# Ajax0564/VyomAI

Measured on AMD Instinct MI355X. Metric: training tokens/sec (12L d=768 seq=512 GPT-style decoder, CLM), higher is better.
Workload: dtype bf16; 1 GPU; configs[1]: GPT-style Decoder 12L d=768 h=12 RoPE vocab 50265, CLM training B=32/GPU seq=512, AdamW, bf16 kernels + fp32 masters; global_batch=32, seq_len=512, parallelism=dp1, attention=none, weights=deterministic recipe (vyomai_amd.recipe)

## Files before the change

### vyomai_amd/csrc/vy_misc.hip

```cpp
#include "vy_common.h"
#include <stdarg.h>
#include <string.h>

static thread_local char g_err[512] = "";
void vy_set_error(const char* fmt, ...) {
  va_list ap;
  va_start(ap, fmt);
  vsnprintf(g_err, sizeof(g_err), fmt, ap);
  va_end(ap);
}
extern "C" const char* vy_last_error(void) { return g_err; }
extern "C" int vy_abi_version(void) { return 5; }

namespace {

template <typename T, int CH>
__global__ __launch_bounds__(256) void layernorm_fwd_kernel(const T* __restrict__ x, int64_t ldx,
                                                            const T* __restrict__ gamma,
                                                            const T* __restrict__ beta, T* __restrict__ y,
                                                            int64_t ldy, float* __restrict__ mean_out,
                                                            float* __restrict__ rstd_out, int64_t M, int N,
                                                            float eps) {
  constexpr int VEC = Chunk<T>::VEC;
  const int lane = threadIdx.x & 63;
  const int64_t row = (int64_t)blockIdx.x * 4 + (threadIdx.x >> 6);
  if (row >= M) return;
  const int nch = N / VEC;
  float v[CH][VEC];
  float s = 0.f;
#pragma unroll
  for (int c = 0; c < CH; ++c) {
    const int ch = lane + 64 * c;
    if (ch < nch) {
      Chunk<T>::load(x + row * ldx + (int64_t)ch * VEC, v[c]);
#pragma unroll
      for (int e = 0; e < VEC; ++e) s += v[c][e];
    } else {
#pragma unroll
      for (int e = 0; e < VEC; ++e) v[c][e] = 0.f;
    }
  }
  const float mean = vy_wave_sum(s) / (float)N;
  float q = 0.f;
#pragma unroll
  for (int c = 0; c < CH; ++c) {
    const int ch = lane + 64 * c;
    if (ch < nch) {
#pragma unroll
      for (int e = 0; e < VEC; ++e) { const float d = v[c][e] - mean; q += d * d; }
    }
  }
  const float var = vy_wave_sum(q) / (float)N;
  const float rstd = rsqrtf(var + eps);
  const float rstd_r = rstd * (1.5f - 0.5f * (var + eps) * rstd * rstd);
#pragma unroll
  for (int c = 0; c < CH; ++c) {
    const int ch = lane + 64 * c;
    if (ch < nch) {
      float g[VEC], b[VEC], o[VEC];
      Chunk<T>::load(gamma + (int64_t)ch * VEC, g);
      Chunk<T>::load(beta + (int64_t)ch * VEC, b);
#pragma unroll
      for (int e = 0; e < VEC; ++e) o[e] = (v[c][e] - mean) * rstd_r * g[e] + b[e];
      Chunk<T>::store(y + row * ldy + (int64_t)ch * VEC, o);
    }
  }
  if (lane == 0) {
    if (mean_out) mean_out[row] = mean;
    if (rstd_out) rstd_out[row] = rstd_r;
  }
}

template <typename T, int CH>
__global__ __launch_bounds__(256) void rmsnorm_fwd_kernel(const T* __restrict__ x, int64_t ldx,
                                                          const T* __restrict__ w, T* __restrict__ y, int64_t ldy,
                                                          int64_t M, int N, float eps, float w_offset) {
  constexpr int VEC = Chunk<T>::VEC;
  const int lane = threadIdx.x & 63;
  const int64_t row = (int64_t)blockIdx.x * 4 + (threadIdx.x >> 6);
  if (row >= M) return;
  const int nch = N / VEC;
  float v[CH][VEC];
  float q = 0.f;
#pragma unroll
  for (int c = 0; c < CH; ++c) {
    const int ch = lane + 64 * c;
    if (ch < nch) {
      Chunk<T>::load(x + row * ldx + (int64_t)ch * VEC, v[c]);
#pragma unroll
      for (int e = 0; e < VEC; ++e) q += v[c][e] * v[c][e];
    }
  }
  const float ms = vy_wave_sum(q) / (float)N + eps;
  float r = rsqrtf(ms);
  r = r * (1.5f - 0.5f * ms * r * r);
#pragma unroll
  for (int c = 0; c < CH; ++c) {
    const int ch = lane + 64 * c;
    if (ch < nch) {
      float g[VEC], o[VEC];
      Chunk<T>::load(w + (int64_t)ch * VEC, g);
#pragma unroll
      for (int e = 0; e < VEC; ++e) o[e] = v[c][e] * r * (w_offset + g[e]);
      Chunk<T>::store(y + row * ldy + (int64_t)ch * VEC, o);
    }
  }
}

template <typename T, int ACT>
__global__ void gated_act_kernel(const T* __restrict__ gu, int64_t ldg, T* __restrict__ out, int64_t ldo,
                                 int64_t M, int I, int code) {
  constexpr int VEC = Chunk<T>::VEC;
  const int nch = I / VEC;
  const int64_t total = M * nch;
  vy_act_dispatch<ACT>(code, [&](auto a_) {
    constexpr int A = decltype(a_)::value;
    for (int64_t i = (int64_t)blockIdx.x * blockDim.x + threadIdx.x; i < total; i += (int64_t)gridDim.x * blockDim.x) {
      const int64_t m = i / nch;
      const int c = (int)(i - m * nch) * VEC;
      float a[VEC], b[VEC], o[VEC];
      Chunk<T>::load(gu + m * ldg + c, a);
      Chunk<T>::load(gu + m * ldg + I + c, b);
#pragma unroll
      for (int e = 0; e < VEC; ++e) {
        if constexpr (ACT == VY_ACT_RUNTIME && sizeof(T) == 2) o[e] = vy_act_fwd_fast<A>(a[e]) * b[e];
        else o[e] = vy_act_fwd<A>(a[e]) * b[e];
      }
      Chunk<T>::store(out + m * ldo + c, o);
    }
  });
}

template <typename T, int CH>
__global__ __launch_bounds__(256) void layernorm_bwd_kernel(
    const T* __restrict__ dy, int64_t lddy, const T* __restrict__ x, int64_t ldx,
    const T* __restrict__ gamma, const float* __restrict__ mean, const float* __restrict__ rstd,
    T* __restrict__ dx, int64_t lddx, float* __restrict__ ws, int64_t M, int N, int W) {
  constexpr int VEC = Chunk<T>::VEC;
  const int lane = threadIdx.x & 63;
  const int wid = blockIdx.x * 4 + (threadIdx.x >> 6);
  const int nch = N / VEC;
  float g[CH][VEC], dg[CH][VEC], db[CH][VEC];
#pragma unroll
  for (int c = 0; c < CH; ++c) {
    const int ch = lane + 64 * c;
#pragma unroll
    for (int e = 0; e < VEC; ++e) { dg[c][e] = 0.f; db[c][e] = 0.f; g[c][e] = 0.f; }
    if (ch < nch) Chunk<T>::load(gamma + (int64_t)ch * VEC, g[c]);
  }
  typedef typename Chunk<T>::Raw Raw;
  Raw xr[CH], dr[CH], xn[CH], dn[CH];
  float mu = 0.f, rs = 0.f, mu_n = 0.f, rs_n = 0.f;
  auto fetch = [&](int64_t row, Raw (&xa)[CH], Raw (&da)[CH], float& m_, float& r_) {
    m_ = mean[row]; r_ = rstd[row];
#pragma unroll
    for (int c = 0; c < CH; ++c) {
      const int ch = lane + 64 * c;
      if (ch < nch) {
        xa[c] = *reinterpret_cast<const Raw*>(x + row * ldx + (int64_t)ch * VEC);
        da[c] = *reinterpret_cast<const Raw*>(dy + row * lddy + (int64_t)ch * VEC);
      }
    }
  };
  if (wid < M) fetch(wid, xr, dr, mu, rs);
  for (int64_t row = wid; row < M; row += W) {
    const bool more = row + W < M;
    if (more) fetch(row + W, xn, dn, mu_n, rs_n);
    float xh[CH][VEC], gy[CH][VEC];
    float s1 = 0.f, s2 = 0.f;
#pragma unroll
    for (int c = 0; c < CH; ++c) {
      const int ch = lane + 64 * c;
      if (ch < nch) {
        float xv[VEC], dv[VEC];
        Chunk<T>::unpack(xr[c], xv);
        Chunk<T>::unpack(dr[c], dv);
#pragma unroll
        for (int e = 0; e < VEC; ++e) {
          xh[c][e] = (xv[e] - mu) * rs;
          gy[c][e] = dv[e] * g[c][e];
          s1 += gy[c][e];
          s2 += gy[c][e] * xh[c][e];
          dg[c][e] += dv[e] * xh[c][e];
          db[c][e] += dv[e];
        }
      }
    }
    s1 = vy_wave_sum(s1) / (float)N;
    s2 = vy_wave_sum(s2) / (float)N;
#pragma unroll
    for (int c = 0; c < CH; ++c) {
      const int ch = lane + 64 * c;
      if (ch < nch) {
        float o[VEC];
#pragma unroll
        for (int e = 0; e < VEC; ++e) o[e] = rs * (gy[c][e] - s1 - xh[c][e] * s2);
        Chunk<T>::store(dx + row * lddx + (int64_t)ch * VEC, o);
      }
    }
    if (more) {
#pragma unroll
      for (int c = 0; c < CH; ++c) { xr[c] = xn[c]; dr[c] = dn[c]; }
      mu = mu_n; rs = rs_n;
    }
  }
  __shared__ float red[2][3][64 * CH * VEC];
  const int wv = threadIdx.x >> 6;
  if (wv > 0) {
#pragma unroll
    for (int c = 0; c < CH; ++c)
#pragma unroll
      for (int e = 0; e < VEC; ++e) {
        red[0][wv - 1][(c * VEC + e) * 64 + lane] = dg[c][e];
        red[1][wv - 1][(c * VEC + e) * 64 + lane] = db[c][e];
      }
  }
  __syncthreads();
  if (wv != 0) return;
  const int WB = W / 4;
  float* wg = ws + (int64_t)blockIdx.x * N;
  float* wb = ws + (int64_t)WB * N + (int64_t)blockIdx.x * N;
#pragma unroll
  for (int c = 0; c < CH; ++c) {
    const int ch = lane + 64 * c;
    if (ch < nch) {
#pragma unroll
      for (int e = 0; e < VEC; ++e) {
        float a = dg[c][e], b = db[c][e];
#pragma unroll
        for (int w2 = 0; w2 < 3; ++w2) {
          a += red[0][w2][(c * VEC + e) * 64 + lane];
          b += red[1][w2][(c * VEC + e) * 64 + lane];
        }
        wg[ch * VEC + e] = a; wb[ch * VEC + e] = b;
      }
    }
  }
}

__global__ __launch_bounds__(256) void colsum_partials_kernel(float* __restrict__ ws, int W, int N,
                                                              float* __restrict__ out0, float* __restrict__ out1,
                                                              int rows_per_slice, int acc) {
  __shared__ float red[2][4][64];
  const int c = threadIdx.x & 63, g = threadIdx.x >> 6;
  const int n = blockIdx.x * 64 + c;
  const int w0 = blockIdx.y * rows_per_slice, w1 = min(W, w0 + rows_per_slice);
  float a = 0.f, b = 0.f;
  if (n < N) {
    for (int wb = w0 + g; wb < w1; wb += 32) {
      float av[8], bv[8];
#pragma unroll
      for (int i = 0; i < 8; ++i) {
        const int w = wb + 4 * i;
        const int wc = w < w1 ? w : wb;
        av[i] = ws[(int64_t)wc * N + n];
        bv[i] = ws[(int64_t)(W + wc) * N + n];
      }
#pragma unroll
      for (int i = 0; i < 8; ++i)
        if (wb + 4 * i < w1) { a += av[i]; b += bv[i]; }
    }
  }
  red[0][g][c] = a; red[1][g][c] = b;
  __syncthreads();
  if (g == 0 && n < N && w0 < w1) {
    a = red[0][0][c] + red[0][1][c] + red[0][2][c] + red[0][3][c];
    b = red[1][0][c] + red[1][1][c] + red[1][2][c] + red[1][3][c];
    if (gridDim.y == 1) {
      if (out0) out0[n] = (acc ? out0[n] : 0.f) + a;
      if (out1) out1[n] = (acc ? out1[n] : 0.f) + b;
    } else {
      ws[(int64_t)w0 * N + n] = a;
      ws[(int64_t)(W + w0) * N + n] = b;
    }
  }
}

__global__ __launch_bounds__(256) void colsum_finish_kernel(const float* __restrict__ ws, int W, int N,
                                                            float* __restrict__ out0, float* __restrict__ out1,
                                                            int rows_per_slice, int acc) {
  const int n = blockIdx.x * 256 + threadIdx.x;
  if (n >= N) return;
  float a = 0.f, b = 0.f;
  for (int w = 0; w < W; w += rows_per_slice) {
    a += ws[(int64_t)w * N + n];
    b += ws[(int64_t)(W + w) * N + n];
  }
  if (out0) out0[n] = (acc ? out0[n] : 0.f) + a;
  if (out1) out1[n] = (acc ? out1[n] : 0.f) + b;
}

template <typename T>
__device__ __forceinline__ float rl(float x) { return x; }
template <>
__device__ __forceinline__ float rl<bf16>(float x) { return vy_round_bf16(x); }

template <typename T>
__global__ void rope_kernel(T* __restrict__ x, int64_t sb, int64_t sh, int64_t sl,
                            const float* __restrict__ cos_tab, const float* __restrict__ sin_tab,
                            int64_t pos0, int64_t B, int heads, int64_t L, int dh, int inverse) {
  const int half = dh >> 1;
  const int64_t idx = (int64_t)blockIdx.x * blockDim.x + threadIdx.x;
  const int64_t total = B * heads * L * half;
  if (idx >= total) return;
  const int i = (int)(idx % half);
  int64_t r = idx / half;
  const int64_t l = r % L; r /= L;
  const int hd = (int)(r % heads);
  const int64_t b = r / heads;
  T* p = x + b * sb + hd * sh + l * sl;
  const float c = rl<T>(cos_tab[(pos0 + l) * half + i]);
  float s = rl<T>(sin_tab[(pos0 + l) * half + i]);
  if (inverse) s = -s;
  const float a = VyT<T>::ld(p + i), bb = VyT<T>::ld(p + i + half);
  VyT<T>::st(p + i, rl<T>(a * c) + rl<T>(-bb * s));
  VyT<T>::st(p + i + half, rl<T>(bb * c) + rl<T>(a * s));
}

template <typename T>
__global__ void rope2_kernel(T* __restrict__ xq, int64_t q_sb, int64_t q_sh, int64_t q_sl, int hq,
                             T* __restrict__ xk, int64_t k_sb, int64_t k_sh, int64_t k_sl, int hk,
                             const float* __restrict__ cos_tab, const float* __restrict__ sin_tab,
                             int64_t pos0, int64_t B, int64_t L, int dh) {
  const bool isk = blockIdx.y == 1;
  T* x = isk ? xk : xq;
  const int64_t sb = isk ? k_sb : q_sb, sh = isk ? k_sh : q_sh, sl = isk ? k_sl : q_sl;
  const int heads = isk ? hk : hq;
  const int half = dh >> 1;
  const int64_t idx = (int64_t)blockIdx.x * blockDim.x + threadIdx.x;
  if (idx >= B * heads * L * half) return;
  const int i = (int)(idx % half);
  int64_t r = idx / half;
  const int64_t l = r % L; r /= L;
  const int hd = (int)(r % heads);
  const int64_t b = r / heads;
  T* p = x + b * sb + hd * sh + l * sl;
  const float c = rl<T>(cos_tab[(pos0 + l) * half + i]);
  const float s = rl<T>(sin_tab[(pos0 + l) * half + i]);
  const float a = VyT<T>::ld(p + i), bb = VyT<T>::ld(p + i + half);
  VyT<T>::st(p + i, rl<T>(a * c) + rl<T>(-bb * s));
  VyT<T>::st(p + i + half, rl<T>(bb * c) + rl<T>(a * s));
}

template <typename S, typename D>
__global__ void cast_kernel(const S* __restrict__ src, D* __restrict__ dst, int64_t n) {
  int64_t i = ((int64_t)blockIdx.x * blockDim.x + threadIdx.x) * 4;
  const int64_t stride = (int64_t)gridDim.x * blockDim.x * 4;
  for (; i < n; i += stride) {
#pragma unroll
    for (int e = 0; e < 4; ++e)
      if (i + e < n) dst[i + e] = (D)(float)src[i + e];
  }
}

template <typename T>
__global__ void transpose_kernel(const T* __restrict__ in, int64_t ldin, T* __restrict__ out, int64_t ldout,
// ... 284 lines not shown
    float v[VEC], o[VEC];
    Chunk<T>::load(row + (int64_t)c * VEC, v);
#pragma unroll
    for (int e = 0; e < VEC; ++e) {
      const int col = c * VEC + e;
      float g = 0.f;
      if (!dead && col < V) g = p.grad(s, __expf(v[e] - l), col == label ? 1.f : 0.f);
      o[e] = g;
    }
    Chunk<T>::store(row + (int64_t)c * VEC, o);
  }
}

template <typename P>
__global__ __launch_bounds__(1024) void row_fused_kernel(bf16* __restrict__ logits, int64_t ld,
                                                         const int64_t* __restrict__ labels, const P p,
                                                         float* __restrict__ lse, int V, int* __restrict__ err) {
  constexpr int CPT = 8;
  __shared__ float red[16];
  const int tid = threadIdx.x;
  const int64_t m = blockIdx.x;
  const int64_t label = labels[m];
  const auto s = p.load(m, true);
  bf16* row = logits + m * ld;
  const int nch = (V + 7) / 8;
  bf16x8 zero8;
#pragma unroll
  for (int e = 0; e < 8; ++e) zero8[e] = (bf16)0.f;
  const bool live = p.live(s, label);
  const bool oob = live && (label < 0 || label >= V);
  if (oob && err && tid == 0) *err = 1;
  if (!live || oob) {
    for (int c = tid; c < nch; c += 1024) *reinterpret_cast<bf16x8*>(row + (int64_t)c * 8) = zero8;
    if (tid == 0) { lse[m] = 0.f; p.skip(m); }
    return;
  }
  const float x_label = (float)row[label];
  bf16x8 v[CPT];
#pragma unroll
  for (int i = 0; i < CPT; ++i) {
    const int c = tid + i * 1024;
    if (c < nch) v[i] = *reinterpret_cast<const bf16x8*>(row + (int64_t)c * 8);
  }
  float mx = -INFINITY;
#pragma unroll
  for (int i = 0; i < CPT; ++i) {
    const int c = tid + i * 1024;
    if (c < nch) {
#pragma unroll
      for (int e = 0; e < 8; ++e)
        if (c * 8 + e < V) mx = fmaxf(mx, (float)v[i][e]);
    }
  }
  if constexpr (P::kSample) {
    __shared__ RowBest redb[16];
    RowBest best{-INFINITY, INT32_MAX};
#pragma unroll
    for (int i = 0; i < CPT; ++i) {
      const int c = tid + i * 1024;
      if (c < nch) {
        float f[8];
        Chunk<bf16>::unpack(v[i], f);
        p.template scan<8>(m, c, f, V, best);
      }
    }
    const RowBest g = block_argmax(best, redb);
    if (tid == 0) p.sampled(m, g.col);
  }
  const float gmx = block_reduce(mx, red, true);
  float sm = 0.f;
#pragma unroll
  for (int i = 0; i < CPT; ++i) {
    const int c = tid + i * 1024;
    if (c < nch) {
#pragma unroll
      for (int e = 0; e < 8; ++e)
        if (c * 8 + e < V) sm += __expf((float)v[i][e] - gmx);
    }
  }
  const float gsm = block_reduce(sm, red, false);
  const float l = gmx + __logf(gsm);
  if (tid == 0) {
    lse[m] = l;
    p.emit(m, l, x_label);
  }
#pragma unroll
  for (int i = 0; i < CPT; ++i) {
    const int c = tid + i * 1024;
    if (c < nch) {
      bf16x8 o;
#pragma unroll
      for (int e = 0; e < 8; ++e) {
        const int col = c * 8 + e;
        float g = 0.f;
        if (col < V) g = p.grad(s, __expf((float)v[i][e] - l), col == label ? 1.f : 0.f);
        o[e] = (bf16)g;
      }
      *reinterpret_cast<bf16x8*>(row + (int64_t)c * 8) = o;
    }
  }
}

int row_check(const char* fn, bool ptrs, const void* logits, int64_t ld, int64_t M, int64_t V, int dtype, const char* pair) {
  if (!ptrs || M <= 0 || V <= 0) VY_FAIL(VY_ERR_ARG, "%s: bad arguments", fn);
  if (pair) {
    if (dtype != VY_BF16) VY_FAIL(VY_ERR_UNSUPPORTED, "%s: bf16 only (use %s)", fn, pair);
    if (V > 65536) VY_FAIL(VY_ERR_UNSUPPORTED, "%s: V=%ld exceeds the 65536 columns a workgroup keeps in registers (use %s)", fn, (long)V, pair);
    if (ld % 8 || ld < vy_cdiv(V, 8) * 8 || (uintptr_t)logits % 16) VY_FAIL(VY_ERR_ARG, "%s: rows must be 16-byte aligned and cover the padded width", fn);
    return VY_OK;
  }
  const int vec = dtype == VY_BF16 ? 8 : 4;
  if (ld % vec || ld < vy_cdiv(V, vec) * vec) VY_FAIL(VY_ERR_ARG, "%s: row stride must be a multiple of %d and cover the padded row", fn, vec);
  if (dtype != VY_BF16 && dtype != VY_F32) VY_FAIL(VY_ERR_ARG, "%s: bad dtype %d", fn, dtype);
  return VY_OK;
}

template <typename P>
int row_lse(const char* fn, bool ptrs, const void* logits, int64_t ld, const int64_t* labels, const P& p, float* lse,
            int64_t M, int64_t V, int32_t* err, int dtype, void* stream) {
  if (const int rc = row_check(fn, ptrs && logits && labels && lse, logits, ld, M, V, dtype, nullptr)) return rc;
  const dim3 grid((unsigned)M), block(256);
  if (dtype == VY_BF16) hipLaunchKernelGGL((row_lse_kernel<bf16, P>), grid, block, 0, (hipStream_t)stream, (const bf16*)logits, ld, labels, p, lse, (int)V, err);
  else hipLaunchKernelGGL((row_lse_kernel<float, P>), grid, block, 0, (hipStream_t)stream, (const float*)logits, ld, labels, p, lse, (int)V, err);
  VY_CHECK_LAUNCH(fn);
  return VY_OK;
}

template <typename P>
int row_grad(const char* fn, bool ptrs, void* logits, int64_t ld, const int64_t* labels, const P& p, const float* lse,
             int64_t M, int64_t V, int dtype, void* stream) {
  if (const int rc = row_check(fn, ptrs && logits && labels && lse, logits, ld, M, V, dtype, nullptr)) return rc;
  const dim3 grid((unsigned)M), block(256);
  if (dtype == VY_BF16) hipLaunchKernelGGL((row_grad_kernel<bf16, P>), grid, block, 0, (hipStream_t)stream, (bf16*)logits, ld, labels, p, lse, (int)V);
  else hipLaunchKernelGGL((row_grad_kernel<float, P>), grid, block, 0, (hipStream_t)stream, (float*)logits, ld, labels, p, lse, (int)V);
  VY_CHECK_LAUNCH(fn);
  return VY_OK;
}

template <typename P>
int row_fused(const char* fn, bool ptrs, void* logits, int64_t ld, const int64_t* labels, const P& p, float* lse,
              int64_t M, int64_t V, int32_t* err, int dtype, void* stream) {
  if (const int rc = row_check(fn, ptrs && logits && labels && lse, logits, ld, M, V, dtype, P::kPair)) return rc;
  hipLaunchKernelGGL((row_fused_kernel<P>), dim3((unsigned)M), dim3(1024), 0, (hipStream_t)stream, (bf16*)logits, ld, labels, p, lse, (int)V, err);
  VY_CHECK_LAUNCH(fn);
  return VY_OK;
}

template <typename T>
int ln_fwd_dispatch(const void* x, int64_t ldx, const void* gamma, const void* beta, void* y, int64_t ldy,
                    float* mean, float* rstd, int64_t M, int64_t N, float eps, hipStream_t st) {
  constexpr int VEC = Chunk<T>::VEC;
  if (N % VEC || ldx % VEC || ldy % VEC) VY_FAIL(VY_ERR_ARG, "vy_layernorm_fwd: N/ld must be multiples of %d", VEC);
  const int nch = (int)(N / VEC);
  const dim3 grid((unsigned)vy_cdiv(M, 4)), block(256);
#define LN_GO(CH)                                                                                       \
  hipLaunchKernelGGL((layernorm_fwd_kernel<T, CH>), grid, block, 0, st, (const T*)x, ldx, (const T*)gamma, \
                     (const T*)beta, (T*)y, ldy, mean, rstd, M, (int)N, eps)
  if (nch <= 64) LN_GO(1);
  else if (nch <= 128) LN_GO(2);
  else if (nch <= 256) LN_GO(4);
  else if (nch <= 512) LN_GO(8);
  else if (nch <= 1024) LN_GO(16);
  else VY_FAIL(VY_ERR_UNSUPPORTED, "vy_layernorm_fwd: N=%ld too wide", (long)N);
#undef LN_GO
  VY_CHECK_LAUNCH("vy_layernorm_fwd");
  return VY_OK;
}

template <typename T>
int ln_bwd_dispatch(const void* dy, int64_t lddy, const void* x, int64_t ldx, const void* gamma,
                    const float* mean, const float* rstd, void* dx, int64_t lddx, float* dgamma,
                    float* dbeta, float beta, float* ws, int64_t M, int64_t N, hipStream_t st, bool partial = false) {
  constexpr int VEC = Chunk<T>::VEC;
  if (N % VEC || ldx % VEC || lddy % VEC || lddx % VEC) VY_FAIL(VY_ERR_ARG, "vy_layernorm_bwd: N/ld must be multiples of %d", VEC);
  const int nch = (int)(N / VEC);
  const int WB = (int)vy_layernorm_bwd_ws_rows(M);
  const int W = WB * 4;
  const dim3 grid((unsigned)WB), block(256);
#define LN_GO(CH)                                                                                        \
  hipLaunchKernelGGL((layernorm_bwd_kernel<T, CH>), grid, block, 0, st, (const T*)dy, lddy, (const T*)x, ldx, \
                     (const T*)gamma, mean, rstd, (T*)dx, lddx, ws, M, (int)N, W)
  if (nch <= 64) LN_GO(1);
  else if (nch <= 128) LN_GO(2);
  else if (nch <= 256) LN_GO(4);
  else VY_FAIL(VY_ERR_UNSUPPORTED, "vy_layernorm_bwd: N=%ld too wide", (long)N);
#undef LN_GO
  VY_CHECK_LAUNCH("vy_layernorm_bwd");
  if (partial) return VY_OK;
  if (beta != 0.f && beta != 1.f) VY_FAIL(VY_ERR_ARG, "vy_layernorm_bwd: beta must be 0 or 1");
  return vy_ln_colsum(ws, WB, (int)N, dgamma, dbeta, beta == 1.f, st);
}

}

int vy_ln_colsum(float* ws, int WB, int N, float* dgamma, float* dbeta, int acc, hipStream_t st) {
  const int slices = vy_ln_colsum_slices(WB);
  const int rps = (int)vy_cdiv(WB, slices);
  hipLaunchKernelGGL(colsum_partials_kernel, dim3((unsigned)vy_cdiv(N, 64), (unsigned)slices), dim3(256), 0, st, ws, WB,
                     N, dgamma, dbeta, rps, acc);
  VY_CHECK_LAUNCH("vy_layernorm_bwd(colsum)");
  if (slices > 1) {
    hipLaunchKernelGGL(colsum_finish_kernel, dim3((unsigned)vy_cdiv(N, 256)), dim3(256), 0, st, ws, WB, N, dgamma,
                       dbeta, rps, acc);
    VY_CHECK_LAUNCH("vy_layernorm_bwd(colsum finish)");
  }
  return VY_OK;
}

extern "C" int vy_layernorm_fwd(const void* x, int64_t ldx, const void* gamma, const void* beta, void* y,
                                int64_t ldy, float* mean, float* rstd, int64_t M, int64_t N, float eps,
                                int dtype, void* stream) {
  if (!x || !gamma || !beta || !y || M <= 0 || N <= 0) VY_FAIL(VY_ERR_ARG, "vy_layernorm_fwd: bad arguments");
  hipStream_t st = (hipStream_t)stream;
  if (dtype == VY_BF16) return ln_fwd_dispatch<bf16>(x, ldx, gamma, beta, y, ldy, mean, rstd, M, N, eps, st);
  if (dtype == VY_F32) return ln_fwd_dispatch<float>(x, ldx, gamma, beta, y, ldy, mean, rstd, M, N, eps, st);
  VY_FAIL(VY_ERR_ARG, "vy_layernorm_fwd: bad dtype %d", dtype);
}

extern "C" int vy_rmsnorm_fwd(const void* x, int64_t ldx, const void* w, void* y, int64_t ldy, int64_t M, int64_t N,
                              float eps, float w_offset, int dtype, void* stream) {
  if (!x || !w || !y || M <= 0 || N <= 0) VY_FAIL(VY_ERR_ARG, "vy_rmsnorm_fwd: bad arguments");
  hipStream_t st = (hipStream_t)stream;
  const int vec = dtype == VY_BF16 ? 8 : 4;
  if (N % vec || ldx % vec || ldy % vec) VY_FAIL(VY_ERR_ARG, "vy_rmsnorm_fwd: N/ld must be multiples of %d", vec);
  const int nch = (int)(N / vec);
  const dim3 grid((unsigned)vy_cdiv(M, 4)), block(256);
#define RMS_GO(T, CH) hipLaunchKernelGGL((rmsnorm_fwd_kernel<T, CH>), grid, block, 0, st, (const T*)x, ldx, (const T*)w, (T*)y, ldy, M, (int)N, eps, w_offset)
#define RMS_DISPATCH(T)                                  \
  if (nch <= 64) RMS_GO(T, 1);                           \
  else if (nch <= 128) RMS_GO(T, 2);                     \
  else if (nch <= 256) RMS_GO(T, 4);                     \
  else if (nch <= 512) RMS_GO(T, 8);                     \
  else if (nch <= 1024) RMS_GO(T, 16);                   \
  else VY_FAIL(VY_ERR_UNSUPPORTED, "vy_rmsnorm_fwd: N=%ld too wide", (long)N)
  if (dtype == VY_BF16) { RMS_DISPATCH(bf16); }
  else if (dtype == VY_F32) { RMS_DISPATCH(float); }
  else VY_FAIL(VY_ERR_ARG, "vy_rmsnorm_fwd: bad dtype %d", dtype);
#undef RMS_DISPATCH
#undef RMS_GO
  VY_CHECK_LAUNCH("vy_rmsnorm_fwd");
  return VY_OK;
}

extern "C" int vy_gated_act_fwd(const void* gate_up, int64_t ldg, void* out, int64_t ldo, int64_t M, int64_t I, int act,
                                int dtype, void* stream) {
  if (!gate_up || !out || M <= 0 || I <= 0) VY_FAIL(VY_ERR_ARG, "vy_gated_act_fwd: bad arguments");
  if (dtype != VY_BF16 && dtype != VY_F32) VY_FAIL(VY_ERR_ARG, "vy_gated_act_fwd: bad dtype %d", dtype);
  if (act != VY_ACT_GELU_ERF && act != VY_ACT_GELU_TANH && !vy_act_is_runtime(act))
    VY_FAIL(VY_ERR_ARG, "vy_gated_act_fwd: unsupported act %d", act);
  hipStream_t st = (hipStream_t)stream;
  const int vec = dtype == VY_BF16 ? 8 : 4;
  if (I % vec || ldg % vec || ldo % vec) VY_FAIL(VY_ERR_ARG, "vy_gated_act_fwd: I/ld must be multiples of %d", vec);
  const int64_t want = vy_cdiv(M * (I / vec), 256);
  const dim3 grid((unsigned)(want < 8192 ? want : 8192)), block(256);
#define GA_GO(T, A) hipLaunchKernelGGL((gated_act_kernel<T, A>), grid, block, 0, st, (const T*)gate_up, ldg, (T*)out, ldo, M, (int)I, act)
  if (dtype == VY_BF16 && act == VY_ACT_GELU_TANH) GA_GO(bf16, VY_ACT_GELU_TANH);
  else if (dtype == VY_BF16 && act == VY_ACT_GELU_ERF) GA_GO(bf16, VY_ACT_GELU_ERF);
  else if (dtype == VY_F32 && act == VY_ACT_GELU_TANH) GA_GO(float, VY_ACT_GELU_TANH);
  else if (dtype == VY_F32 && act == VY_ACT_GELU_ERF) GA_GO(float, VY_ACT_GELU_ERF);
  else if (dtype == VY_BF16) GA_GO(bf16, VY_ACT_RUNTIME);
  else GA_GO(float, VY_ACT_RUNTIME);
#undef GA_GO
  VY_CHECK_LAUNCH("vy_gated_act_fwd");
  return VY_OK;
}

extern "C" int64_t vy_layernorm_bwd_ws_rows(int64_t M) {
  static const int64_t cap = [] { const char* e = getenv("VY_LNBWD_WB"); return e ? (int64_t)atoi(e) : (int64_t)512; }();
  const int64_t b = (M + 3) / 4;
  return b < 1 ? 1 : (b > cap ? cap : b);
}

extern "C" int vy_layernorm_bwd(const void* dy, int64_t lddy, const void* x, int64_t ldx, const void* gamma,
                                const float* mean, const float* rstd, void* dx, int64_t lddx, float* dgamma,
                                float* dbeta, float beta, float* ws, int64_t M, int64_t N, int dtype,
                                void* stream) {
  if (!dy || !x || !gamma || !mean || !rstd || !dx || !ws || M <= 0 || N <= 0)
    VY_FAIL(VY_ERR_ARG, "vy_layernorm_bwd: bad arguments");
  hipStream_t st = (hipStream_t)stream;
  if (dtype == VY_BF16) return ln_bwd_dispatch<bf16>(dy, lddy, x, ldx, gamma, mean, rstd, dx, lddx, dgamma, dbeta, beta, ws, M, N, st);
  if (dtype == VY_F32) return ln_bwd_dispatch<float>(dy, lddy, x, ldx, gamma, mean, rstd, dx, lddx, dgamma, dbeta, beta, ws, M, N, st);
  VY_FAIL(VY_ERR_ARG, "vy_layernorm_bwd: bad dtype %d", dtype);
}

extern "C" int vy_layernorm_bwd_partial(const void* dy, int64_t lddy, const void* x, int64_t ldx, const void* gamma,
                                        const float* mean, const float* rstd, void* dx, int64_t lddx, float* ws,
                                        int64_t M, int64_t N, int dtype, void* stream) {
  if (!dy || !x || !gamma || !mean || !rstd || !dx || !ws || M <= 0 || N <= 0)
    VY_FAIL(VY_ERR_ARG, "vy_layernorm_bwd_partial: bad arguments");
  hipStream_t st = (hipStream_t)stream;
  if (dtype == VY_BF16) return ln_bwd_dispatch<bf16>(dy, lddy, x, ldx, gamma, mean, rstd, dx, lddx, nullptr, nullptr, 0.f, ws, M, N, st, true);
  if (dtype == VY_F32) return ln_bwd_dispatch<float>(dy, lddy, x, ldx, gamma, mean, rstd, dx, lddx, nullptr, nullptr, 0.f, ws, M, N, st, true);
  VY_FAIL(VY_ERR_ARG, "vy_layernorm_bwd_partial: bad dtype %d", dtype);
}

int vy_rope_qk(void* q, int64_t q_sb, int64_t q_sh, int64_t q_sl, int hq, void* k, int64_t k_sb, int64_t k_sh,
               int64_t k_sl, int hk, const float* cos_tab, const float* sin_tab, int64_t pos0, int64_t B, int64_t L, int dh,
               int dtype, hipStream_t st) {
  if (!q || !k || !cos_tab || !sin_tab || (dh & 1)) VY_FAIL(VY_ERR_ARG, "vy_rope_qk: bad arguments");
  const int64_t total = B * (hq > hk ? hq : hk) * L * (dh / 2);
  const dim3 grid((unsigned)vy_cdiv(total, 256), 2), block(256);
  if (dtype == VY_BF16)
    hipLaunchKernelGGL(rope2_kernel<bf16>, grid, block, 0, st, (bf16*)q, q_sb, q_sh, q_sl, hq, (bf16*)k, k_sb, k_sh, k_sl, hk,
                       cos_tab, sin_tab, pos0, B, L, dh);
  else if (dtype == VY_F32)
    hipLaunchKernelGGL(rope2_kernel<float>, grid, block, 0, st, (float*)q, q_sb, q_sh, q_sl, hq, (float*)k, k_sb, k_sh, k_sl,
                       hk, cos_tab, sin_tab, pos0, B, L, dh);
  else VY_FAIL(VY_ERR_ARG, "vy_rope_qk: bad dtype %d", dtype);
  VY_CHECK_LAUNCH("vy_rope_qk");
  return VY_OK;
}

extern "C" int vy_rope_fwd(void* x, int64_t sb, int64_t sh, int64_t sl, const float* cos_tab,
                           const float* sin_tab, int64_t pos0, int64_t B, int heads, int64_t L, int dh,
                           int inverse, int dtype, void* stream) {
  if (!x || !cos_tab || !sin_tab || dh % 2 || B <= 0 || heads <= 0 || L <= 0)
    VY_FAIL(VY_ERR_ARG, "vy_rope_fwd: bad arguments");
  hipStream_t st = (hipStream_t)stream;
  const int64_t total = B * heads * L * (dh / 2);
  const dim3 grid((unsigned)vy_cdiv(total, 256)), block(256);
  if (dtype == VY_BF16)
    hipLaunchKernelGGL(rope_kernel<bf16>, grid, block, 0, st, (bf16*)x, sb, sh, sl, cos_tab, sin_tab, pos0, B, heads, L, dh, inverse);
  else if (dtype == VY_F32)
    hipLaunchKernelGGL(rope_kernel<float>, grid, block, 0, st, (float*)x, sb, sh, sl, cos_tab, sin_tab, pos0, B, heads, L, dh, inverse);
  else VY_FAIL(VY_ERR_ARG, "vy_rope_fwd: bad dtype %d", dtype);
  VY_CHECK_LAUNCH("vy_rope_fwd");
  return VY_OK;
}

extern "C" int vy_act_bwd(const void* dy, int64_t lddy, const void* pre, int64_t ldpre, void* dx, int64_t lddx,
                          int64_t M, int64_t N, int act, int dtype, void* stream) {
  if (!dy || !pre || !dx || M <= 0 || N <= 0) VY_FAIL(VY_ERR_ARG, "vy_act_bwd: bad arguments");
  hipStream_t st = (hipStream_t)stream;
// ... 351 lines not shown
```

Measured before the change: 887,400 tokens/s.

## Process multiple rows per wave in layernorm fwd and deepen bwd prefetch pipeline

The forward LayerNorm kernel now has each wave handle two rows when the row is narrow. It issues all raw loads up front, with clamped addresses so no branch is needed, and interleaves the two reductions to hide latency. The backward kernel replaces single-row double buffering with a D-deep ring of register buffers, clamped speculative fetches and batched per-lane loads of mean/rstd, which are read back with readlane. Both changes aim to hide global memory latency in these memory-bound kernels, at the cost of more registers and possibly lower occupancy.

```diff
diff --git a/vyomai_amd/csrc/vy_misc.hip b/vyomai_amd/csrc/vy_misc.hip
--- a/vyomai_amd/csrc/vy_misc.hip
+++ b/vyomai_amd/csrc/vy_misc.hip
@@ -14,7 +14,9 @@
 
 namespace {
 
-template <typename T, int CH>
+template <int CH> struct LnFwdRows { static constexpr int R = CH <= 4 ? 2 : 1; };
+
+template <typename T, int CH, int R>
 __global__ __launch_bounds__(256) void layernorm_fwd_kernel(const T* __restrict__ x, int64_t ldx,
                                                             const T* __restrict__ gamma,
                                                             const T* __restrict__ beta, T* __restrict__ y,
@@ -22,52 +24,89 @@
                                                             float* __restrict__ rstd_out, int64_t M, int N,
                                                             float eps) {
   constexpr int VEC = Chunk<T>::VEC;
+  typedef typename Chunk<T>::Raw Raw;
   const int lane = threadIdx.x & 63;
-  const int64_t row = (int64_t)blockIdx.x * 4 + (threadIdx.x >> 6);
-  if (row >= M) return;
+  const int64_t row0 = ((int64_t)blockIdx.x * 4 + (threadIdx.x >> 6)) * R;
+  if (row0 >= M) return;
   const int nch = N / VEC;
-  float v[CH][VEC];
-  float s = 0.f;
+  Raw xr[R][CH], gr[CH], br[CH];
 #pragma unroll
   for (int c = 0; c < CH; ++c) {
-    const int ch = lane + 64 * c;
-    if (ch < nch) {
-      Chunk<T>::load(x + row * ldx + (int64_t)ch * VEC, v[c]);
-#pragma unroll
-      for (int e = 0; e < VEC; ++e) s += v[c][e];
-    } else {
-#pragma unroll
-      for (int e = 0; e < VEC; ++e) v[c][e] = 0.f;
-    }
-  }
-  const float mean = vy_wave_sum(s) / (float)N;
-  float q = 0.f;
-#pragma unroll
-  for (int c = 0; c < CH; ++c) {
-    const int ch = lane + 64 * c;
-    if (ch < nch) {
-#pragma unroll
-      for (int e = 0; e < VEC; ++e) { const float d = v[c][e] - mean; q += d * d; }
-    }
-  }
-  const float var = vy_wave_sum(q) / (float)N;
-  const float rstd = rsqrtf(var + eps);
-  const float rstd_r = rstd * (1.5f - 0.5f * (var + eps) * rstd * rstd);
-#pragma unroll
-  for (int c = 0; c < CH; ++c) {
-    const int ch = lane + 64 * c;
-    if (ch < nch) {
-      float g[VEC], b[VEC], o[VEC];
-      Chunk<T>::load(gamma + (int64_t)ch * VEC, g);
-      Chunk<T>::load(beta + (int64_t)ch * VEC, b);
-#pragma unroll
-      for (int e = 0; e < VEC; ++e) o[e] = (v[c][e] - mean) * rstd_r * g[e] + b[e];
-      Chunk<T>::store(y + row * ldy + (int64_t)ch * VEC, o);
-    }
-  }
-  if (lane == 0) {
-    if (mean_out) mean_out[row] = mean;
-    if (rstd_out) rstd_out[row] = rstd_r;
+    const int ch = lane + 64 * c < nch ? lane + 64 * c : nch - 1;
+    gr[c] = *reinterpret_cast<const Raw*>(gamma + (int64_t)ch * VEC);
+    br[c] = *reinterpret_cast<const Raw*>(beta + (int64_t)ch * VEC);
+  }
+#pragma unroll
+  for (int r = 0; r < R; ++r) {
+    const int64_t row = row0 + r < M ? row0 + r : M - 1;
+#pragma unroll
+    for (int c = 0; c < CH; ++c) {
+      const int ch = lane + 64 * c < nch ? lane + 64 * c : nch - 1;
+      xr[r][c] = *reinterpret_cast<const Raw*>(x + row * ldx + (int64_t)ch * VEC);
+    }
+  }
+  float v[R][CH][VEC], mean[R], rstd_r[R];
+#pragma unroll
+  for (int r = 0; r < R; ++r) {
+    float s = 0.f;
+#pragma unroll
+    for (int c = 0; c < CH; ++c) {
+      const int ch = lane + 64 * c;
+      if (ch < nch) {
+        Chunk<T>::unpack(xr[r][c], v[r][c]);
+#pragma unroll
+        for (int e = 0; e < VEC; ++e) s += v[r][c][e];
+      } else {
+#pragma unroll
+        for (int e = 0; e < VEC; ++e) v[r][c][e] = 0.f;
+      }
+    }
+    mean[r] = s;
+  }
+#pragma unroll
+  for (int r = 0; r < R; ++r) mean[r] = vy_wave_sum(mean[r]) / (float)N;
+#pragma unroll
+  for (int r = 0; r < R; ++r) {
+    float q = 0.f;
+#pragma unroll
+    for (int c = 0; c < CH; ++c) {
+      const int ch = lane + 64 * c;
+      if (ch < nch) {
+#pragma unroll
+        for (int e = 0; e < VEC; ++e) { const float d = v[r][c][e] - mean[r]; q += d * d; }
+      }
+    }
+    rstd_r[r] = q;
+  }
+#pragma unroll
+  for (int r = 0; r < R; ++r) {
+    const float var = vy_wave_sum(rstd_r[r]) / (float)N;
+    const float rstd = rsqrtf(var + eps);
+    rstd_r[r] = rstd * (1.5f - 0.5f * (var + eps) * rstd * rstd);
+  }
+#pragma unroll
+  for (int r = 0; r < R; ++r) {
+    const int64_t row = row0 + r;
+    if (row < M) {
+#pragma unroll
+      for (int c = 0; c < CH; ++c) {
+        const int ch = lane + 64 * c;
+        if (ch < nch) {
+          float g[VEC], b[VEC], o[VEC];
+          Chunk<T>::unpack(gr[c], g);
+          Chunk<T>::unpack(br[c], b);
+#pragma unroll
+          for (int e = 0; e < VEC; ++e) o[e] = (v[r][c][e] - mean[r]) * rstd_r[r] * g[e] + b[e];
+          Chunk<T>::store(y + row * ldy + (int64_t)ch * VEC, o);
+        }
+      }
+      if (lane == 0) {
+        if (mean_out) mean_out[row] = mean[r];
+        if (rstd_out) rstd_out[row] = rstd_r[r];
+      }
+    }
+#pragma unroll
+    for (int c = 0; c < CH; ++c) asm volatile("" ::"v"(xr[r][c]));
   }
 }
 
@@ -131,7 +170,7 @@
   });
 }
 
-template <typename T, int CH>
+template <typename T, int CH, int D>
 __global__ __launch_bounds__(256) void layernorm_bwd_kernel(
     const T* __restrict__ dy, int64_t lddy, const T* __restrict__ x, int64_t ldx,
     const T* __restrict__ gamma, const float* __restrict__ mean, const float* __restrict__ rstd,
@@ -149,59 +188,70 @@
     if (ch < nch) Chunk<T>::load(gamma + (int64_t)ch * VEC, g[c]);
   }
   typedef typename Chunk<T>::Raw Raw;
-  Raw xr[CH], dr[CH], xn[CH], dn[CH];
-  float mu = 0.f, rs = 0.f, mu_n = 0.f, rs_n = 0.f;
-  auto fetch = [&](int64_t row, Raw (&xa)[CH], Raw (&da)[CH], float& m_, float& r_) {
-    m_ = mean[row]; r_ = rstd[row];
+  constexpr int NB = D + 1;
+  constexpr int BATCH = 64 / NB * NB;
+  Raw xr[NB][CH], dr[NB][CH];
+  const int64_t last = wid < M ? wid + (M - 1 - wid) / W * W : 0;
+  auto fetch = [&](int64_t row, Raw (&xa)[CH], Raw (&da)[CH]) {
+    const bool real = row < M;
+    row = real ? row : last;
 #pragma unroll
     for (int c = 0; c < CH; ++c) {
-      const int ch = lane + 64 * c;
-      if (ch < nch) {
-        xa[c] = *reinterpret_cast<const Raw*>(x + row * ldx + (int64_t)ch * VEC);
-        da[c] = *reinterpret_cast<const Raw*>(dy + row * lddy + (int64_t)ch * VEC);
-      }
+      const int ch = !real ? 0 : lane + 64 * c < nch ? lane + 64 * c : nch - 1;
+      xa[c] = *reinterpret_cast<const Raw*>(x + row * ldx + (int64_t)ch * VEC);
+      da[c] = *reinterpret_cast<const Raw*>(dy + row * lddy + (int64_t)ch * VEC);
     }
   };
-  if (wid < M) fetch(wid, xr, dr, mu, rs);
-  for (int64_t row = wid; row < M; row += W) {
-    const bool more = row + W < M;
-    if (more) fetch(row + W, xn, dn, mu_n, rs_n);
-    float xh[CH][VEC], gy[CH][VEC];
-    float s1 = 0.f, s2 = 0.f;
-#pragma unroll
-    for (int c = 0; c < CH; ++c) {
-      const int ch = lane + 64 * c;
-      if (ch < nch) {
-        float xv[VEC], dv[VEC];
-        Chunk<T>::unpack(xr[c], xv);
-        Chunk<T>::unpack(dr[c], dv);
-#pragma unroll
-        for (int e = 0; e < VEC; ++e) {
-          xh[c][e] = (xv[e] - mu) * rs;
-          gy[c][e] = dv[e] * g[c][e];
-          s1 += gy[c][e];
-          s2 += gy[c][e] * xh[c][e];
-          dg[c][e] += dv[e] * xh[c][e];
-          db[c][e] += dv[e];
+  for (int64_t b0 = wid; b0 < M; b0 += (int64_t)BATCH * W) {
+    const int64_t srow = b0 + (int64_t)lane * W < M ? b0 + (int64_t)lane * W : last;
+    const float mu_l = mean[srow], rs_l = rstd[srow];
+#pragma unroll
+    for (int s = 0; s < D; ++s) {
+      fetch(b0 + (int64_t)s * W, xr[s], dr[s]);
+      __builtin_amdgcn_sched_barrier(0);
+    }
+    for (int k = 0; k < BATCH && b0 + (int64_t)k * W < M; k += NB) {
+#pragma unroll
+      for (int s = 0; s < NB; ++s) {
+#pragma clang fp contract(off)
+        const int64_t row = b0 + (int64_t)(k + s) * W;
+        fetch(k + s + D < BATCH ? row + (int64_t)D * W : M, xr[(s + D) % NB], dr[(s + D) % NB]);
+        if (row >= M) continue;
+        const float mu = __int_as_float(__builtin_amdgcn_readlane(__float_as_int(mu_l), k + s));
+        const float rs = __int_as_float(__builtin_amdgcn_readlane(__float_as_int(rs_l), k + s));
+        float xh[CH][VEC], gy[CH][VEC];
+        float s1 = 0.f, s2 = 0.f;
+#pragma unroll
+        for (int c = 0; c < CH; ++c) {
+          const int ch = lane + 64 * c;
+          if (ch < nch) {
+            float xv[VEC], dv[VEC];
+            Chunk<T>::unpack(xr[s][c], xv);
+            Chunk<T>::unpack(dr[s][c], dv);
+#pragma unroll
+            for (int e = 0; e < VEC; ++e) {
+              xh[c][e] = (xv[e] - mu) * rs;
+              gy[c][e] = dv[e] * g[c][e];
+              s1 += gy[c][e];
+              s2 += gy[c][e] * xh[c][e];
+              dg[c][e] = fmaf(dv[e], xh[c][e], dg[c][e]);
+              db[c][e] += dv[e];
+            }
+          }
         }
-      }
-    }
-    s1 = vy_wave_sum(s1) / (float)N;
-    s2 = vy_wave_sum(s2) / (float)N;
-#pragma unroll
-    for (int c = 0; c < CH; ++c) {
-      const int ch = lane + 64 * c;
-      if (ch < nch) {
-        float o[VEC];
-#pragma unroll
-        for (int e = 0; e < VEC; ++e) o[e] = rs * (gy[c][e] - s1 - xh[c][e] * s2);
-        Chunk<T>::store(dx + row * lddx + (int64_t)ch * VEC, o);
-      }
-    }
-    if (more) {
-#pragma unroll
-      for (int c = 0; c < CH; ++c) { xr[c] = xn[c]; dr[c] = dn[c]; }
-      mu = mu_n; rs = rs_n;
+        s1 = vy_wave_sum(s1) / (float)N;
+        s2 = vy_wave_sum(s2) / (float)N;
+#pragma unroll
+        for (int c = 0; c < CH; ++c) {
+          const int ch = lane + 64 * c;
+          if (ch < nch) {
+            float o[VEC];
+#pragma unroll
+            for (int e = 0; e < VEC; ++e) o[e] = rs * fmaf(-s2, xh[c][e], gy[c][e] - s1);
+            Chunk<T>::store(dx + row * lddx + (int64_t)ch * VEC, o);
+          }
+        }
+      }
     }
   }
   __shared__ float red[2][3][64 * CH * VEC];
@@ -792,10 +842,10 @@
   constexpr int VEC = Chunk<T>::VEC;
   if (N % VEC || ldx % VEC || ldy % VEC) VY_FAIL(VY_ERR_ARG, "vy_layernorm_fwd: N/ld must be multiples of %d", VEC);
   const int nch = (int)(N / VEC);
-  const dim3 grid((unsigned)vy_cdiv(M, 4)), block(256);
-#define LN_GO(CH)                                                                                       \
-  hipLaunchKernelGGL((layernorm_fwd_kernel<T, CH>), grid, block, 0, st, (const T*)x, ldx, (const T*)gamma, \
-                     (const T*)beta, (T*)y, ldy, mean, rstd, M, (int)N, eps)
+  const dim3 block(256);
+#define LN_GO(CH)                                                                                                      \
+  hipLaunchKernelGGL((layernorm_fwd_kernel<T, CH, LnFwdRows<CH>::R>), dim3((unsigned)vy_cdiv(M, 4 * LnFwdRows<CH>::R)), \
+                     block, 0, st, (const T*)x, ldx, (const T*)gamma, (const T*)beta, (T*)y, ldy, mean, rstd, M, (int)N, eps)
   if (nch <= 64) LN_GO(1);
   else if (nch <= 128) LN_GO(2);
   else if (nch <= 256) LN_GO(4);
@@ -818,7 +868,7 @@
   const int W = WB * 4;
   const dim3 grid((unsigned)WB), block(256);
 #define LN_GO(CH)                                                                                        \
-  hipLaunchKernelGGL((layernorm_bwd_kernel<T, CH>), grid, block, 0, st, (const T*)dy, lddy, (const T*)x, ldx, \
+  hipLaunchKernelGGL((layernorm_bwd_kernel<T, CH, (CH <= 2 ? 2 : 1)>), grid, block, 0, st, (const T*)dy, lddy, (const T*)x, ldx, \
                      (const T*)gamma, mean, rstd, (T*)dx, lddx, ws, M, (int)N, W)
   if (nch <= 64) LN_GO(1);
   else if (nch <= 128) LN_GO(2);
```

After: 890,200 tokens/s (median of 6 runs). Within noise of the previous version (+0.3%).
